# locuslab/lcp-physics

Measured on NVIDIA H100. Metric: LCP solves/sec (LCPFunction fwd+bwd, batch=4096 x 64 contacts, fp32), higher is better.
Workload: dtype f32 I/O and iterates; the condensed n x n KKT matrix is formed, factored and solved in f64

## Files before the change

lcp_physics_b200/csrc/lcp_condensed.cuh:

```cuda
#pragma once
#include "lcp_device.cuh"

namespace lcpb200 {
namespace cnd {

constexpr int NT = 256;
constexpr int UC = 8;
constexpr int CSMAX = 6;
constexpr int KS = 8;
constexpr int LMAX = 16;
constexpr int LU_BW = 2;
constexpr int MISC_BAND_LU = 4;
constexpr int CFLAG_DENSE_LU = 4;
constexpr int STATUS_UNSUPPORTED = -100;

struct CPlan {
  int ok;
  int n, m, e, N, NP, NS;
  int pcap;
  int wcap;
  int smem_bytes;
  int ctas_per_sm;
  int flags;
  int sbytes;
// ... 307 lines not shown
      S.clist()[rank * n + a] = (unsigned short)v;
    }
    if (l == 0) S.clcnt()[a] = (unsigned char)cnt;
  }
  __syncthreads();
  return true;
}

template <typename T>
struct EngineSoA {
  const T *mass, *inertia, *v, *fext;
  const T *normal, *p1, *p2;
  const T *mu, *rest;
  const int32_t *b1, *b2;
  const int32_t* nc_s;
  int nb, nc;
  int mode;
  T dt;
  T *p_s, *h_s;
};

template <typename T>
__device__ __forceinline__ void contact_row(T p1x, T p1y, T p2x, T p2y, T dx, T dy, T (&r1)[3], T (&r2)[3]) {
  r1[0] = p1x * dy - p1y * dx; r1[1] = dx; r1[2] = dy;
  r2[0] = -(p2x * dy - p2y * dx); r2[1] = -dx; r2[2] = -dy;
}

template <typename T>
__device__ __noinline__ bool build_structure_soa(const CPlan& P, CSmem<T>& S, Struct& st, const EngineSoA<T>& e_,
                                                 int sc, const T* __restrict__ A, int* singular) {
  const int n = P.n, e = P.e, tid = threadIdx.x, pcap = P.pcap;
  const int nb = e_.nb, ncs = e_.nc, cs = e_.mode == 0 ? 4 : 1;
  const int nc = e_.nc_s ? e_.nc_s[sc] : e_.nc;
  const int m = cs * nc;
  const int32_t* tb1 = e_.b1 + (e_.nc_s ? (size_t)sc * ncs : 0);
  const int32_t* tb2 = e_.b2 + (e_.nc_s ? (size_t)sc * ncs : 0);
  char* sb = reinterpret_cast<char*>(S.K());
  unsigned short* cl_tmp = reinterpret_cast<unsigned short*>(sb);
  int* cl_cnt = reinterpret_cast<int*>(sb + al16((size_t)LMAX * n * 2));
  if (n != 3 * nb || nc < 0 || nc > ncs || m > P.m || nc * cs > pcap || nc * cs * cs > P.wcap) return false;
  const T* mass = e_.mass + (size_t)sc * nb;
  const T* inertia = e_.inertia + (size_t)sc * nb;
  const T* v = e_.v + (size_t)sc * n;
  const T* normal = e_.normal + (size_t)sc * ncs * 2;
  const T* p1 = e_.p1 + (size_t)sc * ncs * 2;
  const T* p2 = e_.p2 + (size_t)sc * ncs * 2;
  T* ps = e_.p_s + (size_t)sc * n;
  T* hs = e_.h_s + (size_t)sc * P.m;
  int bad = 0;
  for (int j = tid; j < n; j += NT) {
    const int body = j / 3;
    const T q = (j - 3 * body == 0) ? inertia[body] : mass[body];
    S.qd()[j] = q;
    if (!(q != T(0) && isfinite((double)q))) bad |= 2;
    ps[j] = e_.mode == 0 ? q * v[j] + e_.dt * e_.fext[(size_t)sc * n + j] : T(0);
    cl_cnt[j] = 0;
  }
  for (int t = tid; t < e * n; t += NT) S.As()[t] = A[t];
  st.ncomp = nc; st.cs = cs; st.m = m;
  st.sh = 0;
  while ((1 << st.sh) < nc) ++st.sh;
  for (int t = tid; t < UC * pcap; t += NT) { S.Gd()[t] = T(0); S.ccols()[t] = 0; }
  for (int t = tid; t < nc * cs * cs; t += NT) S.Fd()[t] = T(0);
  __syncthreads();
  for (int c = tid; c < nc; c += NT) {
    const int b1 = tb1[c], b2 = tb2[c];
    if (b1 == b2 || b1 < 0 || b2 < 0 || b1 >= nb) { bad |= 1; continue; }
    const bool two = b2 < nb;
    const int lo = two ? min(b1, b2) : b1, hi = max(b1, b2);
    const int o1 = b1 < b2 ? 0 : 3, o2 = 3 - o1;
#pragma unroll
    for (int q = 0; q < 3; ++q) {
      S.ccols()[q * pcap + c] = (unsigned char)(3 * lo + q);
      if (two) S.ccols()[(3 + q) * pcap + c] = (unsigned char)(3 * hi + q);
    }
    S.ncols()[c] = two ? 6 : 3;
    const T nx = normal[2 * c], ny = normal[2 * c + 1];
    const T p1x = p1[2 * c], p1y = p1[2 * c + 1], p2x = p2[2 * c], p2y = p2[2 * c + 1];
    T r1[3], r2[3];
    contact_row<T>(p1x, p1y, p2x, p2y, nx, ny, r1, r2);
    const T v20 = two ? v[3 * b2] : T(0), v21 = two ? v[3 * b2 + 1] : T(0), v22 = two ? v[3 * b2 + 2] : T(0);
    const T jv = r1[0] * v[3 * b1] + r1[1] * v[3 * b1 + 1] + r1[2] * v[3 * b1 + 2] +
                 r2[0] * v20 + r2[1] * v21 + r2[2] * v22;
    const T rc = e_.rest[(size_t)sc * ncs + c];
#pragma unroll
    for (int q = 0; q < 3; ++q) { S.Gd()[(size_t)(o1 + q) * pcap + c] = r1[q]; if (two) S.Gd()[(size_t)(o2 + q) * pcap + c] = r2[q]; }
    S.rows()[c] = (unsigned short)c;
    S.posof()[c] = (unsigned short)c;
    if (e_.mode == 0) {
      hs[c] = jv * rc;
      contact_row<T>(p1x, p1y, p2x, p2y, ny, -nx, r1, r2);
#pragma unroll
      for (int q = 0; q < 3; ++q) {
        S.Gd()[(size_t)(o1 + q) * pcap + nc + c] = r1[q];
        S.Gd()[(size_t)(o1 + q) * pcap + 2 * nc + c] = -r1[q];
        if (two) { S.Gd()[(size_t)(o2 + q) * pcap + nc + c] = r2[q]; S.Gd()[(size_t)(o2 + q) * pcap + 2 * nc + c] = -r2[q]; }
      }
      const int rw[4] = {c, nc + 2 * c, nc + 2 * c + 1, 3 * nc + c};
#pragma unroll
      for (int r = 0; r < 4; ++r) { S.rows()[r * nc + c] = (unsigned short)rw[r]; S.posof()[rw[r]] = (unsigned short)(r * nc + c); }
      hs[nc + 2 * c] = T(0); hs[nc + 2 * c + 1] = T(0); hs[3 * nc + c] = T(0);
      S.Fd()[(size_t)(1 * 4 + 3) * nc + c] = T(1);
      S.Fd()[(size_t)(2 * 4 + 3) * nc + c] = T(1);
      S.Fd()[(size_t)(3 * 4 + 0) * nc + c] = e_.mu[(size_t)sc * ncs + c];
      S.Fd()[(size_t)(3 * 4 + 1) * nc + c] = T(-1);
      S.Fd()[(size_t)(3 * 4 + 2) * nc + c] = T(-1);
    } else {
      hs[c] = jv + jv * -rc;
    }
    for (int q = 0; q < (two ? 6 : 3); ++q) {
      const int a = q < 3 ? 3 * lo + q : 3 * hi + q - 3;
      const int slot = atomicAdd(&cl_cnt[a], 1);
      if (slot < LMAX) cl_tmp[slot * n + a] = (unsigned short)(c * 8 + q); else bad |= 1;
    }
  }
  const int anybad = __syncthreads_or(bad);
  if (anybad & 2) { *singular = 1; return false; }
  if (anybad & 1) return false;
  for (int t = tid; t < n * LMAX; t += NT) {
    const int a = t % n, l = t / n, cnt = cl_cnt[a];
    if (l < cnt) {
      const int val = cl_tmp[l * n + a];
      int rank = 0;
      for (int u = 0; u < cnt; ++u) rank += (cl_tmp[u * n + a] < val);
      S.clist()[rank * n + a] = (unsigned short)val;
    }
    if (l == 0) S.clcnt()[a] = (unsigned char)cnt;
  }
  __syncthreads();
  return true;
}

template <typename T>
__device__ __noinline__ void mark_band_lu(const CPlan& P, CSmem<T> S, Struct st) {
  int wide = P.e > 0 || (P.flags & CFLAG_DENSE_LU);
  for (int c = threadIdx.x; c < st.ncomp; c += NT) {
    const int nc = S.ncols()[c];
    if (nc > 0 && (S.ccols()[(nc - 1) * P.pcap + c] >> 4) - (S.ccols()[c] >> 4) > LU_BW) wide = 1;
  }
  wide = __syncthreads_or(wide);
  if (threadIdx.x == 0) S.misc()[MISC_BAND_LU] = !wide;
}

__device__ __forceinline__ double rcp64_fast(double x) {
  double r;
  asm("rcp.approx.ftz.f64 %0, %1;" : "=d"(r) : "d"(x));
  const double ax = fabs(x);
  if (!(ax > 1e-290 && ax < 1e290)) return 1.0 / x;
  r = fma(r, fma(-x, r, 1.0), r);
  r = fma(r, fma(-x, r, 1.0), r);
  return r;
}

template <typename T, int CS>
__device__ __forceinline__ void comp_inverse(const CPlan& P, CSmem<T>& S, const Struct& st) {
  const int nc_ = st.ncomp;
  for (int c = threadIdx.x; c < nc_; c += NT) {
    double M[CS][CS];
#pragma unroll
    for (int r = 0; r < CS; ++r) {
      const int i = S.rows()[r * nc_ + c];
#pragma unroll
      for (int q = 0; q < CS; ++q) M[r][q] = (double)S.Fd()[(size_t)(r * CS + q) * nc_ + c];
      M[r][r] += (i == 0xFFFF) ? 1.0 : ((P.flags & 1) ? 1.0 / (double)S.d()[i] : (double)(T(1) / S.d()[i]));
    }
    unsigned swaps = 0;
    int bit = 0;
#pragma unroll
    for (int k = 0; k < CS; ++k) {
#pragma unroll
      for (int i = k + 1; i < CS; ++i) {
        const bool sw = fabs(M[i][k]) > fabs(M[k][k]);
        swaps |= (sw ? 1u : 0u) << bit;
        ++bit;
#pragma unroll
        for (int q = 0; q < CS; ++q) { const double u = M[k][q], w = M[i][q]; M[k][q] = sw ? w : u; M[i][q] = sw ? u : w; }
      }
      const double r = rcp64_fast(M[k][k]);
      M[k][k] = 1.0;
#pragma unroll
      for (int q = 0; q < CS; ++q) M[k][q] *= r;
#pragma unroll
      for (int i = 0; i < CS; ++i) {
        if (i == k) continue;
        const double f = M[i][k];
        M[i][k] = 0.0;
#pragma unroll
        for (int q = 0; q < CS; ++q) M[i][q] = fma(-f, M[k][q], M[i][q]);
      }
    }
#pragma unroll
    for (int k = CS - 1; k >= 0; --k) {
#pragma unroll
      for (int i = CS - 1; i > k; --i) {
        --bit;
        const bool sw = (swaps >> bit) & 1u;
#pragma unroll
        for (int q = 0; q < CS; ++q) { const double u = M[q][k], w = M[q][i]; M[q][k] = sw ? w : u; M[q][i] = sw ? u : w; }
      }
    }
#pragma unroll
    for (int r = 0; r < CS; ++r)
#pragma unroll
      for (int q = 0; q < CS; ++q) S.W()[(size_t)(r * CS + q) * nc_ + c] = M[r][q];
  }
}

template <int CS>
struct ApplySpan {
  static constexpr int ceil_log2(int x) { return x <= 1 ? 0 : 1 + ceil_log2((x + 1) / 2); }
  static constexpr int U = ((CS << ceil_log2(4 * NT / CS)) + NT - 1) / NT;
};

template <typename T, int CS>
__device__ __forceinline__ void comp_apply(CSmem<T>& S, const Struct& st, bool trans = false) {
  constexpr int U = ApplySpan<CS>::U;
  const int nc_ = st.ncomp;
  const int npos = nc_ * CS;
  const int sh = st.sh, cmask = (1 << sh) - 1, tot = CS << sh;
  double val[U];
#pragma unroll
  for (int u = 0; u < U; ++u) {
    const int t = threadIdx.x + u * NT, r = t >> sh, c = t & cmask;
    val[u] = 0.0;
    if (t < tot && c < nc_) {
      double a = 0.0;
#pragma unroll
      for (int q = 0; q < CS; ++q) a = fma(S.W()[(size_t)(trans ? (q * CS + r) : (r * CS + q)) * nc_ + c], S.scr()[q * nc_ + c], a);
      val[u] = a;
    }
  }
  __syncthreads();
#pragma unroll
  for (int u = 0; u < U; ++u) {
    const int t = threadIdx.x + u * NT, r = t >> sh, c = t & cmask;
    if (t < tot && c < nc_) S.scr()[r * nc_ + c] = val[u];
  }
  (void)npos;
}

template <typename T, int NS, int CS>
__device__ __forceinline__ void assemble_K(const CPlan& P, CSmem<T>& S, const Struct& st) {
  const int nc_ = st.ncomp;
  constexpr int NP = 16 * NS;
  const int n = P.n, N = P.N, e = P.e, tid = threadIdx.x, pcap = P.pcap;
  double* K = S.K();
  {
    double2* K2 = reinterpret_cast<double2*>(K);
    for (int t = tid; t < NP * NP / 2; t += NT) K2[t] = make_double2(0.0, 0.0);
  }
  __syncthreads();
  for (int i = tid; i < NP; i += NT) K[(size_t)i * NP + i] = i < n ? (double)S.qd()[i] : (i < N ? 0.0 : 1.0);
  for (int t = tid; t < e * n; t += NT) {
    const int k = t / n, i = t - k * n;
    const double v = (double)S.As()[t];
    K[(size_t)(n + k) * NP + i] = v;
    K[(size_t)i * NP + n + k] = v;
  }
  __syncthreads();
  const int grp = tid >> 3, q2 = tid & 7;
  for (int a0 = 0; a0 < n; a0 += NT / 8) {
    const int a = a0 + grp;
    const int cnt = a < n ? (int)S.clcnt()[a] : 0;
    int mx = cnt;
    mx = max(mx, __shfl_xor_sync(FULL, mx, 8));
    mx = max(mx, __shfl_xor_sync(FULL, mx, 16));
    for (int l = 0; l < mx; ++l) {
      if (l < cnt) {
        const int cp = S.clist()[l * n + a], c = cp >> 3, p = cp & 7;
        if (q2 < (int)S.ncols()[c]) {
          double acc = 0.0;
#pragma unroll
          for (int q = 0; q < CS; ++q) {
            double u = 0.0;
#pragma unroll
            for (int r = 0; r < CS; ++r)
              u = fma((double)S.Gd()[(size_t)p * pcap + r * nc_ + c], S.W()[(size_t)(r * CS + q) * nc_ + c], u);
            acc = fma(u, (double)S.Gd()[(size_t)q2 * pcap + q * nc_ + c], acc);
          }
          K[(size_t)S.ccols()[q2 * pcap + c] * NP + a] += acc;
        }
      }
      __syncwarp();
    }
  }
  __syncthreads();
}

template <int NS, int BW>
struct LuBand {
  static constexpr bool DENSE = BW >= NS - 1;
  static constexpr int W = DENSE ? NS : 2 * BW + 1;
  static __device__ __forceinline__ constexpr bool in(int r, int c) { return DENSE || (r - c <= BW && c - r <= BW); }
  static __device__ __forceinline__ constexpr int col(int r, int c) { return DENSE ? c : c - r + BW; }
  static __host__ __device__ constexpr int end(int b0) { return DENSE || b0 + BW + 1 > NS ? NS : b0 + BW + 1; }
};

template <int NS, int BW, int B0>
__device__ __forceinline__ void lu_phase(double (&a)[NS][LuBand<NS, BW>::W], int o_buf, int o_rdiag, int& step, int ti,
                                         int tj) {
  using Bd = LuBand<NS, BW>;
  constexpr int NP = 16 * NS;
  constexpr int E = Bd::end(B0);
  constexpr int L = E - B0;
  constexpr int CW = (L <= 4) ? L : 3;
  double* const rdiag = reinterpret_cast<double*>(cnd_smem + o_rdiag);
#pragma unroll 1
  for (int kk = 0; kk < 16; kk += 2) {
    const int k = 16 * B0 + kk;
    double2* const U2 = reinterpret_cast<double2*>(cnd_smem + o_buf) + (size_t)(step & 1) * 2 * NP;
    double2* const C2 = U2 + NP;
    ++step;
    {
      const int sr = ti - kk, sc = tj - kk;
      if ((unsigned)sr < 2u) {
        double* dst = reinterpret_cast<double*>(U2) + sr;
#pragma unroll
        for (int c = B0; c < E; ++c) dst[2 * (16 * c + tj)] = a[B0][Bd::col(B0, c)];
      }
      if ((unsigned)sc < 2u) {
        double* dst = reinterpret_cast<double*>(C2) + sc;
#pragma unroll
        for (int r = B0; r < E; ++r) dst[2 * (16 * r + ti)] = a[r][Bd::col(r, B0)];
      }
    }
    __syncthreads();
    const double2 pk = U2[k], pk1 = U2[k + 1];
    const double p01 = pk1.x;
    const double r0 = rcp64_fast(pk.x);
    const double r1 = pk.x * rcp64_fast(fma(pk.x, pk1.y, -(pk.y * p01)));
    const double l10 = pk.y * r0;
    if ((ti | tj) == 0) { rdiag[k] = r0; rdiag[k + 1] = r1; }
#pragma unroll
    for (int cg = B0; cg < E; cg += CW) {
      double w0[CW], w1[CW];
#pragma unroll
      for (int q = 0; q < CW; ++q) {
        const int c = cg + q;
        if (c < E) {
          const double2 u = U2[16 * c + tj];
          const double x1 = fma(-l10, u.x, u.y);
          w0[q] = (c == B0 && !(tj > kk)) ? 0.0 : u.x;
          w1[q] = (c == B0 && !(tj > kk + 1)) ? 0.0 : x1;
        }
      }
#pragma unroll
      for (int r = B0; r < E; ++r) {
        const double2 cc = C2[16 * r + ti];
        double m0 = cc.x * r0;
        double m1 = fma(-m0, p01, cc.y) * r1;
        if (r == B0) {
          m0 = (ti > kk) ? m0 : 0.0;
          m1 = (ti > kk + 1) ? m1 : 0.0;
        }
#pragma unroll
        for (int q = 0; q < CW; ++q) {
          const int c = cg + q;
          if (c < E) a[r][Bd::col(r, c)] = fma(-m1, w1[q], fma(-m0, w0[q], a[r][Bd::col(r, c)]));
        }
      }
    }
  }
}

template <int NS, int BW, int B0>
struct LuPhases {
  static __device__ __forceinline__ void run(double (&a)[NS][LuBand<NS, BW>::W], int o_buf, int o_rdiag, int& step, int ti,
                                             int tj) {
    lu_phase<NS, BW, B0>(a, o_buf, o_rdiag, step, ti, tj);
    LuPhases<NS, BW, B0 + 1>::run(a, o_buf, o_rdiag, step, ti, tj);
  }
};
template <int NS, int BW>
struct LuPhases<NS, BW, NS> {
  static __device__ __forceinline__ void run(double (&)[NS][LuBand<NS, BW>::W], int, int, int&, int, int) {}
};

template <int NS> struct SolveLayout {
  static constexpr int NP = 16 * NS;
  static constexpr int QN = (NP + 31) / 32;
  static constexpr int ROUNDS = NP / QN;
  static constexpr size_t BYTES = (size_t)ROUNDS * QN * QN * 32 * 8;
};

template <int NS, int BW>
__device__ __forceinline__ void factor_K_body(int o_K, int o_rdiag, bool trans) {
  using Bd = LuBand<NS, BW>;
  constexpr int NP = 16 * NS, QN = SolveLayout<NS>::QN;
  int tid_;
  asm volatile("mov.u32 %0, %%tid.x;" : "=r"(tid_));
  const int ti = tid_ & 15, tj = tid_ >> 4;
  double* const K = reinterpret_cast<double*>(cnd_smem + o_K);
  double* const rdiag = reinterpret_cast<double*>(cnd_smem + o_rdiag);
  double a[NS][Bd::W];
#pragma unroll
  for (int c = 0; c < NS; ++c)
#pragma unroll
    for (int r = 0; r < NS; ++r)
      if (Bd::in(r, c)) a[r][Bd::col(r, c)] = K[(size_t)(16 * c + tj) * NP + 16 * r + ti];
  __syncthreads();
  int step = 0;
  LuPhases<NS, BW, 0>::run(a, o_K, o_rdiag, step, ti, tj);
  __syncthreads();
  int rowpart[NS];
  double rrow[NS];
#pragma unroll
  for (int r = 0; r < NS; ++r) {
    const int i = 16 * r + ti;
    rowpart[r] = trans ? (i / QN) * QN * QN * 32 + (i % QN) * 32 : (i % QN) * QN * 32 + i / QN;
    rrow[r] = rdiag[i];
  }
#pragma unroll
  for (int c = 0; c < NS; ++c) {
    const int j = 16 * c + tj;
    const double rj = rdiag[j];
    const int colpart = trans ? (j % QN) * QN * 32 + j / QN : (j / QN) * QN * QN * 32 + (j % QN) * 32;
#pragma unroll
    for (int r = 0; r < NS; ++r) {
      const int i = 16 * r + ti;
      const double v = Bd::in(r, c) ? a[r][Bd::col(r, c)] : 0.0;
      K[colpart + rowpart[r]] = (i != j) ? v * (trans ? rrow[r] : rj) : v;
    }
  }
  __syncthreads();
}

template <int NS>
__device__ __noinline__ void factor_K(int o_K, int o_rdiag, bool trans, bool band) {
  if constexpr (LU_BW < NS - 1) {
    if (band) {
      factor_K_body<NS, LU_BW>(o_K, o_rdiag, trans);
      return;
    }
  }
  factor_K_body<NS, NS - 1>(o_K, o_rdiag, trans);
}

template <int QN>
struct SolveCoef {
  double dg[QN * QN];
  double rw[QN * QN];
};

template <int QN>
__device__ __forceinline__ void solve_load(SolveCoef<QN>& c, const double* blk, int r, int lane) {
#pragma unroll
  for (int t = 0; t < QN * QN; ++t) { c.dg[t] = blk[t * 32 + r]; c.rw[t] = blk[t * 32 + lane]; }
}

template <int QN>
__device__ __forceinline__ void solve_round_fwd(double (&y)[QN], const SolveCoef<QN>& c, int r, int lane) {
  double v[QN];
#pragma unroll
  for (int q = 0; q < QN; ++q) v[q] = __shfl_sync(FULL, y[q], r);
#pragma unroll
  for (int q = 0; q < QN; ++q)
#pragma unroll
    for (int qp = q + 1; qp < QN; ++qp) v[qp] = fma(-c.dg[qp * QN + q], v[q], v[qp]);
  const bool below = lane > r, own = lane == r;
#pragma unroll
  for (int qp = 0; qp < QN; ++qp) {
    double t = y[qp];
#pragma unroll
    for (int q = 0; q < QN; ++q) t = fma(-c.rw[qp * QN + q], v[q], t);
    y[qp] = below ? t : (own ? v[qp] : y[qp]);
  }
}

template <int QN>
__device__ __forceinline__ void solve_round_bwd(double (&y)[QN], const SolveCoef<QN>& c, int r, int lane) {
  double v[QN];
#pragma unroll
  for (int q = 0; q < QN; ++q) v[q] = __shfl_sync(FULL, y[q], r);
#pragma unroll
  for (int q = QN - 1; q >= 0; --q)
#pragma unroll
    for (int qp = q - 1; qp >= 0; --qp) v[qp] = fma(-c.dg[qp * QN + q], v[q], v[qp]);
  const bool above = lane < r, own = lane == r;
#pragma unroll
  for (int qp = 0; qp < QN; ++qp) {
    double t = y[qp];
#pragma unroll
    for (int q = QN - 1; q >= 0; --q) t = fma(-c.rw[qp * QN + q], v[q], t);
    y[qp] = above ? t : (own ? v[qp] : y[qp]);
  }
}

template <int NS>
__device__ __noinline__ void solve_warp(int o_K, int o_rdiag, int o_bx) {
  constexpr int NP = 16 * NS, QN = SolveLayout<NS>::QN, ROUNDS = SolveLayout<NS>::ROUNDS;
  constexpr int STRIDE = QN * QN * 32;
  static_assert(ROUNDS % 2 == 0, "the software pipeline handles two rounds per trip");
  const int lane = threadIdx.x & 31;
  const double* const S = reinterpret_cast<const double*>(cnd_smem + o_K);
  const double* const rdiag = reinterpret_cast<const double*>(cnd_smem + o_rdiag);
  double* const bx = reinterpret_cast<double*>(cnd_smem + o_bx);
  double y[QN];
#pragma unroll
  for (int q = 0; q < QN; ++q) y[q] = (QN * lane + q < NP) ? bx[QN * lane + q] : 0.0;
  SolveCoef<QN> c0, c1;
  solve_load<QN>(c0, S, 0, lane);
#pragma unroll 1
  for (int r = 0; r < ROUNDS; r += 2) {
    solve_load<QN>(c1, S + (size_t)(r + 1) * STRIDE, r + 1, lane);
    solve_round_fwd<QN>(y, c0, r, lane);
    const int rn = (r + 2 < ROUNDS) ? r + 2 : ROUNDS - 1;
    solve_load<QN>(c0, S + (size_t)rn * STRIDE, rn, lane);
    solve_round_fwd<QN>(y, c1, r + 1, lane);
  }
#pragma unroll 1
  for (int r = ROUNDS - 1; r > 0; r -= 2) {
    solve_load<QN>(c1, S + (size_t)(r - 1) * STRIDE, r - 1, lane);
    solve_round_bwd<QN>(y, c0, r, lane);
    const int rn = (r - 2 >= 0) ? r - 2 : 0;
    solve_load<QN>(c0, S + (size_t)rn * STRIDE, rn, lane);
    solve_round_bwd<QN>(y, c1, r - 1, lane);
  }
#pragma unroll
  for (int q = 0; q < QN; ++q) {
    const int i = QN * lane + q;
    if (i < NP) bx[i] = y[q] * rdiag[i];
  }
}

template <typename T, int CS, int NS, typename PF>
__device__ __noinline__ void solve_kkt(const CPlan& P, CSmem<T> S, Struct st, PF& pf, const T* rx,
                                       const T* rs, const T* rz, const T* ry, T* dx, T* ds, T* dz, T* dy,
                                       bool trans = false) {
  const int nc_ = st.ncomp;
  const int n = P.n, e = P.e, N = P.N, NP = P.NP, tid = threadIdx.x, pcap = P.pcap;
  const int npos = st.ncomp * CS;
  for (int p = tid; p < npos; p += NT) {
    const int i = S.rows()[p];
    double t = 0.0;
    if (i != 0xFFFF) t = (P.flags & 2) ? ((double)(rz ? rz[i] : T(0)) - (double)rs[i] / (double)S.d()[i]) : (double)((rz ? rz[i] : T(0)) - rs[i] / S.d()[i]);
    S.scr()[p] = t;
  }
  __syncthreads();
  comp_apply<T, CS>(S, st, trans);
  __syncthreads();
  for (int a = tid; a < NP; a += NT) {
    double acc = 0.0;
    if (a < n) {
      const int cnt = S.clcnt()[a];
      for (int l = 0; l < cnt; ++l) {
        const int cp = S.clist()[l * n + a], c = cp >> 3, p = cp & 7;
#pragma unroll
        for (int r = 0; r < CS; ++r) acc = fma((double)S.Gd()[(size_t)p * pcap + r * nc_ + c], S.scr()[r * nc_ + c], acc);
      }
      acc = -(double)(rx ? rx[a] : T(0)) - acc;
    } else if (a < N) {
      acc = -(double)(ry ? ry[a - n] : T(0));
    }
    S.bx()[a] = acc;
  }
  __syncthreads();
  pf.lap(CPH_SOLVE_RHS);
  if (tid < 32) solve_warp<NS>(P.o_K, P.o_rdiag, P.o_bx);
  __syncthreads();
  pf.lap(CPH_SOLVE_TRI);
  for (int tt = tid; tt < (CS << st.sh); tt += NT) {
    const int c = tt & ((1 << st.sh) - 1);
    if (c >= nc_) continue;
    const int p = (tt >> st.sh) * nc_ + c;
    const int i = S.rows()[p];
    double t = 0.0;
    if (i != 0xFFFF) {
      const int nc = S.ncols()[c];
      t = (P.flags & 2) ? ((double)(rz ? rz[i] : T(0)) - (double)rs[i] / (double)S.d()[i]) : (double)((rz ? rz[i] : T(0)) - rs[i] / S.d()[i]);
      for (int q = 0; q < nc; ++q) t = fma((double)S.Gd()[(size_t)q * pcap + p], S.bx()[S.ccols()[q * pcap + c]], t);
    }
    S.scr()[p] = t;
  }
  __syncthreads();
  comp_apply<T, CS>(S, st, trans);
  __syncthreads();
  for (int p = tid; p < npos; p += NT) {
    const int i = S.rows()[p];
    if (i == 0xFFFF) continue;
    const T wz = (T)S.scr()[p];
    const T rsi = rs[i];
    dz[i] = wz;
    ds[i] = (-rsi - wz) / S.d()[i];
  }
  for (int a = tid; a < n; a += NT) dx[a] = (T)S.bx()[a];
  for (int k = tid; k < e; k += NT) dy[k] = (T)S.bx()[n + k];
  __syncthreads();
  pf.lap(CPH_SOLVE_POST);
}

template <typename T, int NS, int CS, typename PF>
__device__ __noinline__ void factor_kkt(const CPlan& P, CSmem<T> S, Struct st, PF& pf, bool trans = false) {
  comp_inverse<T, CS>(P, S, st);
  __syncthreads();
  pf.lap(CPH_WINV);
  assemble_K<T, NS, CS>(P, S, st);
  pf.lap(CPH_ASSEMBLE);
  if constexpr (LU_BW < NS - 1) factor_K<NS>(P.o_K, P.o_rdiag, trans, S.misc()[MISC_BAND_LU] != 0);
  else factor_K<NS>(P.o_K, P.o_rdiag, trans, false);
  pf.lap(CPH_LU);
}

template <typename T>
__device__ __forceinline__ void get_steps(const T* z, const T* dz, const T* s, const T* ds, int m, T* red, T& step_z,
                                          T& step_s) {
  const T NEG_INF = -INFINITY, POS_INF = INFINITY;
  T mx[2] = {NEG_INF, NEG_INF};
  T mn[2] = {POS_INF, POS_INF};
  T any[2] = {T(0), T(0)};
  for (int i = threadIdx.x; i < m; i += NT) {
    const T az = -z[i] / dz[i], as = -s[i] / ds[i];
    mx[0] = nan_max(mx[0], az);
    mx[1] = nan_max(mx[1], as);
    if (dz[i] > T(0)) any[0] = T(1); else mn[0] = nan_min(mn[0], az);
    if (ds[i] > T(0)) any[1] = T(1); else mn[1] = nan_min(mn[1], as);
  }
  T v[6] = {mx[0], mx[1], -mn[0], -mn[1], any[0], any[1]};
  block_reduce<T, 6>(v, OpMax(), NEG_INF, red);
  const T fz = (v[0] > T(1)) ? v[0] : T(1);
  const T fs = (v[1] > T(1)) ? v[1] : T(1);
  step_z = (v[4] > T(0)) ? nan_min(-v[2], fz) : -v[2];
  step_s = (v[5] > T(0)) ? nan_min(-v[3], fs) : -v[3];
}

template <typename T>
struct CFwdArgs {
  CPlan P;
  int B;
  const T *Q, *p, *G, *h, *A, *b, *F;
  T *zhat, *nu, *lam, *slack, *resid;
  int *status, *iters;
  T eps;
  int not_improved_lim, max_iter;
  long long* prof;
  EngineSoA<T> soa;
  unsigned char* ssave;
};

template <typename T>
struct CBwdArgs {
  CPlan P;
  int B;
  int R, chunks;
  const T *Q, *G, *A, *F;
  const T *zhat, *nu, *lam, *slack, *g;
  T *dQ, *dp, *dG, *dh, *dA, *db, *dF;
  int* done;
  const int* only;
  unsigned flags;
  const unsigned char* sload;
  EngineSoA<T> soa;
  T *dmass, *dinertia, *dv, *dfext, *dnormal, *dp1, *dp2, *dmu, *drest;
  long long* prof;
};

__device__ __forceinline__ void copy16(unsigned char* dst, const unsigned char* src, int bytes) {
  const uint4* s4 = reinterpret_cast<const uint4*>(src);
  uint4* d4 = reinterpret_cast<uint4*>(dst);
  for (int i = threadIdx.x; i < (bytes >> 4); i += NT) d4[i] = s4[i];
}

__device__ __forceinline__ void save_structure(const CPlan& P, const Struct& st, bool ok, unsigned char* dst) {
  if (threadIdx.x == 0) *reinterpret_cast<int4*>(dst) = make_int4(ok ? st.ncomp : -1, st.cs, st.sh, st.m);
  if (!ok) return;
  const int c1 = P.o_x - P.o_Fd, c2 = P.o_y - P.o_qd, c3 = P.o_misc - P.o_rows;
  copy16(dst + 16, cnd_smem + P.o_Fd, c1);
  copy16(dst + 16 + c1, cnd_smem + P.o_qd, c2);
  copy16(dst + 16 + c1 + c2, cnd_smem + P.o_rows, c3);
}

__device__ __forceinline__ bool load_structure(const CPlan& P, Struct& st, const unsigned char* src) {
  const int4 hd = *reinterpret_cast<const int4*>(src);
  st.ncomp = hd.x; st.cs = hd.y; st.sh = hd.z; st.m = hd.w;
  if (hd.x < 0) return false;
  const int c1 = P.o_x - P.o_Fd, c2 = P.o_y - P.o_qd, c3 = P.o_misc - P.o_rows;
  copy16(cnd_smem + P.o_Fd, src + 16, c1);
  copy16(cnd_smem + P.o_qd, src + 16 + c1, c2);
  copy16(cnd_smem + P.o_rows, src + 16 + c1 + c2, c3);
  return true;
}

template <typename T>
struct SzResid { T sz, resid; };

template <typename T, int CS>
__device__ __noinline__ SzResid<T> fwd_residuals(const CFwdArgs<T>& a, CSmem<T> S, Struct st, int sc) {
  const int nc_ = st.ncomp;
  const CPlan& P = a.P;
  const int n = P.n, m = st.m, e = P.e, tid = threadIdx.x, pcap = P.pcap;
  const T* p = a.p + (size_t)sc * n;
  const T* h = a.h + (size_t)sc * P.m;
  const T* b = e > 0 ? a.b + (size_t)sc * e : nullptr;
  for (int c = tid; c < n; c += NT) {
    T acc = 0;
    const int cnt = S.clcnt()[c];
    for (int l = 0; l < cnt; ++l) {
      const int cp = S.clist()[l * n + c], cc = cp >> 3, pp = cp & 7;
#pragma unroll
      for (int r = 0; r < CS; ++r) {
        const int i = S.rows()[r * nc_ + cc];
        if (i != 0xFFFF) acc = fma(S.Gd()[(size_t)pp * pcap + r * nc_ + cc], S.z()[i], acc);
      }
    }
    for (int k = 0; k < e; ++k) acc = fma(S.As()[k * n + c], S.y()[k], acc);
    S.rx()[c] = acc + S.qd()[c] * S.x()[c] + p[c];
  }
  for (int tt = tid; tt < (CS << st.sh); tt += NT) {
    const int r = tt >> st.sh, c = tt & ((1 << st.sh) - 1);
    if (c >= nc_) continue;
    const int pz = r * nc_ + c;
    const int i = S.rows()[pz];
    if (i == 0xFFFF) continue;
    const int nc = S.ncols()[c];
    T acc = 0;
    for (int q = 0; q < nc; ++q) acc = fma(S.Gd()[(size_t)q * pcap + pz], S.x()[S.ccols()[q * pcap + c]], acc);
    T fz = 0;
#pragma unroll
    for (int q = 0; q < CS; ++q) {
      const int j = S.rows()[q * nc_ + c];
      if (j != 0xFFFF) fz = fma(S.Fd()[(size_t)(r * CS + q) * nc_ + c], S.z()[j], fz);
    }
    S.rz()[i] = acc + S.s()[i] - h[i] - fz;
  }
  for (int k = tid; k < e; k += NT) {
    T acc = 0;
    for (int j = 0; j < n; ++j) acc = fma(S.As()[k * n + j], S.x()[j], acc);
    S.ry()[k] = acc - b[k];
  }
  __syncthreads();
  T q4[4] = {0, 0, 0, 0};
  for (int i = tid; i < m; i += NT) { q4[0] += S.s()[i] * S.z()[i]; q4[1] += S.rz()[i] * S.rz()[i]; }
  for (int i = tid; i < e; i += NT) q4[2] += S.ry()[i] * S.ry()[i];
  for (int i = tid; i < n; i += NT) q4[3] += S.rx()[i] * S.rx()[i];
  block_reduce<T, 4>(q4, OpSum(), T(0), S.red());
  const T sz = q4[0];
  const T mu = fabs(sz / T(m));
  return {sz, (e > 0 ? sqrt(q4[2]) : T(0)) + sqrt(q4[1]) + sqrt(q4[3]) + T(m) * mu};
}

template <typename T>
__device__ __noinline__ void fwd_store_best(const CFwdArgs<T>& a, CSmem<T> S, int m, int sc) {
  const CPlan& P = a.P;
  const int n = P.n, e = P.e, tid = threadIdx.x;
  for (int i = tid; i < n; i += NT) a.zhat[(size_t)sc * n + i] = S.x()[i];
  for (int i = tid; i < m; i += NT) { a.lam[(size_t)sc * P.m + i] = S.z()[i]; a.slack[(size_t)sc * P.m + i] = S.s()[i]; }
  for (int i = tid; i < e; i += NT) a.nu[(size_t)sc * e + i] = S.y()[i];
}

template <typename T>
__device__ __noinline__ void fwd_centering(CSmem<T> S, int m, T mu, T sz) {
  const int tid = threadIdx.x;
  T stz, sts;
  get_steps(S.z(), S.dz(), S.s(), S.ds(), m, S.red(), stz, sts);
  const T alpha_aff = nan_min(nan_min(stz, sts), T(1));
  T t3[1] = {0};
  for (int i = tid; i < m; i += NT) t3[0] += (S.s()[i] + alpha_aff * S.ds()[i]) * (S.z()[i] + alpha_aff * S.dz()[i]);
  block_reduce<T, 1>(t3, OpSum(), T(0), S.red());
  const T ratio = t3[0] / sz;
  const T sig = ratio * ratio * ratio;
  const T musig = -mu * sig;
  for (int i = tid; i < m; i += NT) S.rs2()[i] = (musig + S.ds()[i] * S.dz()[i]) / S.s()[i];
  __syncthreads();
}

template <typename T>
__device__ __noinline__ void fwd_step(const CPlan& P, CSmem<T> S, int m) {
  const int n = P.n, e = P.e, tid = threadIdx.x;
  for (int i = tid; i < n; i += NT) S.dx()[i] += S.rx()[i];
  for (int i = tid; i < m; i += NT) { S.ds()[i] += S.rz()[i]; S.dz()[i] += S.rs2()[i]; }
  for (int i = tid; i < e; i += NT) S.dy()[i] += S.ry()[i];
  __syncthreads();
  T stz, sts;
  get_steps(S.z(), S.dz(), S.s(), S.ds(), m, S.red(), stz, sts);
  const T alpha = nan_min(T(0.999) * nan_min(stz, sts), T(1));
  for (int i = tid; i < n; i += NT) S.x()[i] += alpha * S.dx()[i];
  for (int i = tid; i < m; i += NT) { S.s()[i] += alpha * S.ds()[i]; S.z()[i] += alpha * S.dz()[i]; }
  for (int i = tid; i < e; i += NT) S.y()[i] += alpha * S.dy()[i];
  __syncthreads();
}

template <typename T, int NS, int CS, typename PF>
__device__ __forceinline__ void forward_scene(const CFwdArgs<T>& a, CSmem<T>& S, const Struct& st, PF& pf, int sc) {
  const CPlan& P = a.P;
  const int m = st.m;
  {
    const int n = P.n, e = P.e, tid = threadIdx.x;
    const T* h = a.h + (size_t)sc * P.m;
    const T* b = e > 0 ? a.b + (size_t)sc * e : nullptr;
    for (int i = tid; i < m; i += NT) { S.d()[i] = T(1); S.rs2()[i] = T(0); S.rz()[i] = -h[i]; }
    for (int i = tid; i < n; i += NT) S.rx()[i] = a.p[(size_t)sc * n + i];
    for (int i = tid; i < e; i += NT) S.ry()[i] = -b[i];
    __syncthreads();
  }
  factor_kkt<T, NS, CS>(P, S, st, pf);
  solve_kkt<T, CS, NS>(P, S, st, pf, S.rx(), S.rs2(), S.rz(), P.e > 0 ? S.ry() : nullptr, S.x(), S.s(), S.z(), S.y());
  if (m == 0) {
    fwd_store_best<T>(a, S, 0, sc);
    if (threadIdx.x == 0) { a.status[sc] = 2; a.iters[sc] = 0; if (a.resid) a.resid[sc] = T(0); }
    return;
  }
  {
    const int tid = threadIdx.x;
    T mn[2] = {INFINITY, INFINITY};
    for (int i = tid; i < m; i += NT) { mn[0] = nan_min(mn[0], S.s()[i]); mn[1] = nan_min(mn[1], S.z()[i]); }
    block_reduce<T, 2>(mn, OpMin(), (T)INFINITY, S.red());
    for (int i = tid; i < m; i += NT) {
      if (mn[0] <= T(0)) S.s()[i] -= mn[0] - T(1);
      if (mn[1] <= T(0)) S.z()[i] -= mn[1] - T(1);
    }
    __syncthreads();
  }

  T best = nan("");
  bool have_best = false;
  int not_improved = 0, status = 0, it = 0;
  for (it = 0; it < a.max_iter; ++it) {
    const SzResid<T> r = fwd_residuals<T, CS>(a, S, st, sc);
    pf.lap(CPH_RESID);
    const T mu = fabs(r.sz / T(m));

    bool improved;
    if (!have_best) { improved = true; have_best = true; not_improved = 0; }
    else { improved = r.resid < best; not_improved = improved ? 0 : not_improved + 1; }
    if (improved) {
      best = r.resid;
      fwd_store_best<T>(a, S, m, sc);
    }
    if (not_improved == a.not_improved_lim) { status = 1; ++it; break; }
    if (best < a.eps) { status = 2; ++it; break; }
    if (mu > T(1e100)) { status = 3; ++it; break; }

    for (int i = threadIdx.x; i < m; i += NT) S.d()[i] = S.z()[i] / S.s()[i];
    __syncthreads();
    factor_kkt<T, NS, CS>(P, S, st, pf);

    solve_kkt<T, CS, NS>(P, S, st, pf, S.rx(), S.z(), S.rz(), P.e > 0 ? S.ry() : nullptr, S.dx(), S.ds(), S.dz(), S.dy());
    fwd_centering<T>(S, m, mu, r.sz);
    pf.lap(CPH_STEP);
    solve_kkt<T, CS, NS>(P, S, st, pf, nullptr, S.rs2(), nullptr, nullptr, S.rx(), S.rz(), S.rs2(), S.ry());
    fwd_step<T>(P, S, m);
    pf.lap(CPH_STEP);
  }
  if (threadIdx.x == 0) { a.status[sc] = status; a.iters[sc] = it; if (a.resid) a.resid[sc] = best; }
}

template <typename T, int NS, bool PROF>
__global__ void __launch_bounds__(NT, (NS <= 6) ? 2 : 1) cond_forward_kernel(const __grid_constant__ CFwdArgs<T> a) {
  const CPlan& P = a.P;
  CSmem<T> S(P);
  const int n = P.n, m = P.m, e = P.e, tid = threadIdx.x;
  __shared__ int singular_s;
  const T NANV = nan("");
  Prof<PROF> pf(PROF ? a.prof + (size_t)blockIdx.x * CPH_COUNT : nullptr);
  for (int sc = blockIdx.x; sc < a.B; sc += gridDim.x) {
    if (tid == 0) singular_s = 0;
    __syncthreads();
    pf.start();
    Struct st;
    const bool ok = a.soa.mass
        ? build_structure_soa<T>(P, S, st, a.soa, sc, e > 0 ? a.A + (size_t)sc * e * n : nullptr, &singular_s)
        : build_structure<T>(P, S, st, a.Q + (size_t)sc * n * n, a.G + (size_t)sc * m * n,
                             e > 0 ? a.A + (size_t)sc * e * n : nullptr, a.F + (size_t)sc * m * m, &singular_s);
    __syncthreads();
    if (a.ssave) save_structure(P, st, ok, a.ssave + (size_t)sc * P.sbytes);
    pf.lap(CPH_STRUCT);
    if (!ok) {
      if (singular_s) {
        for (int i = tid; i < n; i += NT) a.zhat[(size_t)sc * n + i] = NANV;
        for (int i = tid; i < m; i += NT) { a.lam[(size_t)sc * m + i] = NANV; a.slack[(size_t)sc * m + i] = NANV; }
        for (int i = tid; i < e; i += NT) a.nu[(size_t)sc * e + i] = NANV;
        if (tid == 0) { a.status[sc] = -1; a.iters[sc] = 0; if (a.resid) a.resid[sc] = NANV; }
      } else if (tid == 0) {
        a.status[sc] = STATUS_UNSUPPORTED;
        a.iters[sc] = 0;
      }
      __syncthreads();
      continue;
    }
    if constexpr (LU_BW < NS - 1) mark_band_lu<T>(P, S, st);
    switch (st.cs) {
      case 1: forward_scene<T, NS, 1>(a, S, st, pf, sc); break;
      case 2: forward_scene<T, NS, 2>(a, S, st, pf, sc); break;
      case 3: forward_scene<T, NS, 3>(a, S, st, pf, sc); break;
      case 4: forward_scene<T, NS, 4>(a, S, st, pf, sc); break;
      case 5: forward_scene<T, NS, 5>(a, S, st, pf, sc); break;
      default: forward_scene<T, NS, 6>(a, S, st, pf, sc); break;
    }
    __syncthreads();
  }
}

template <typename T, typename F>
__device__ __forceinline__ void write_outer(T* __restrict__ o, int rows, int cols, F f) {
  constexpr int V = 16 / (int)sizeof(T);
  const int tid = threadIdx.x;
  if (cols % V == 0 && (reinterpret_cast<size_t>(o) & 15) == 0) {
    const int cv = cols / V, total = rows * cv;
    const int di = NT / cv, dj = NT - di * cv;
    int i = tid / cv, jv = tid - i * cv;
    for (int t = tid; t < total; t += NT) {
      const int j = jv * V;
      if (V == 4) {
        float4 w;
        w.x = (float)f(i, j); w.y = (float)f(i, j + 1); w.z = (float)f(i, j + 2); w.w = (float)f(i, j + 3);
        reinterpret_cast<float4*>(o)[t] = w;
      } else {
        double2 w;
        w.x = (double)f(i, j); w.y = (double)f(i, j + 1);
        reinterpret_cast<double2*>(o)[t] = w;
      }
      i += di; jv += dj;
      if (jv >= cv) { jv -= cv; ++i; }
    }
  } else {
    int i = tid / cols, j = tid - i * cols;
    const int di = NT / cols, dj = NT - di * cols;
    for (size_t t = tid; t < (size_t)rows * cols; t += NT) {
      o[t] = f(i, j);
      i += di; j += dj;
      if (j >= cols) { j -= cols; ++i; }
    }
  }
}

template <typename T, int CS, typename PF>
__device__ __forceinline__ void backward_grads(const CBwdArgs<T>& a, CSmem<T>& S, const Struct& st, PF& pf, int sc, int so) {
  const CPlan& P = a.P;
  const int n = P.n, m = st.m, e = P.e, tid = threadIdx.x;
  const T* dx = S.dx(); const T* dlam = S.dz(); const T* dnu = S.dy();
  if (a.soa.mass) {
    const EngineSoA<T>& E = a.soa;
    const int nc = st.ncomp, nb = E.nb, ncs = E.nc;
    const int32_t* tb1 = E.b1 + (E.nc_s ? (size_t)sc * ncs : 0);
    const int32_t* tb2 = E.b2 + (E.nc_s ? (size_t)sc * ncs : 0);
    const T* v = E.v + (size_t)sc * n;
    const T* zh_ = S.x(); const T* lm = S.z();
    for (int c = tid; c < ncs; c += NT) {
      const size_t ic = (size_t)sc * ncs + c, oc = (size_t)so * ncs + c;
      if (c >= nc) {
        if (a.dnormal) { a.dnormal[oc * 2] = 0; a.dnormal[oc * 2 + 1] = 0; }
        if (a.dp1) { a.dp1[oc * 2] = 0; a.dp1[oc * 2 + 1] = 0; }
        if (a.dp2) { a.dp2[oc * 2] = 0; a.dp2[oc * 2 + 1] = 0; }
        if (a.drest) a.drest[oc] = 0;
        if (a.dmu) a.dmu[oc] = 0;
        continue;
      }
      const T nx = E.normal[ic * 2], ny = E.normal[ic * 2 + 1];
      const T p1x = E.p1[ic * 2], p1y = E.p1[ic * 2 + 1], p2x = E.p2[ic * 2], p2y = E.p2[ic * 2 + 1];
      const bool two = tb2[c] < nb;
      const int j1 = 3 * tb1[c], j2 = two ? 3 * tb2[c] : j1;
      const T rc = E.rest[ic];
      const T dhc = -dlam[c] * (E.mode == 0 ? T(1) : T(1));
      T gnx = 0, gny = 0, g1x = 0, g1y = 0, g2x = 0, g2y = 0, jcv = 0;
      const int nrows = E.mode == 0 ? 3 : 1;
      const int rows_[3] = {c, nc + 2 * c, nc + 2 * c + 1};
      const T dxs[3] = {nx, ny, -ny}, dys[3] = {ny, -nx, nx};
      for (int q = 0; q < nrows; ++q) {
        const T ddx_ = dxs[q], ddy_ = dys[q];
        const int i = rows_[q];
        T g[6];
        for (int t = 0; t < 3; ++t) {
          g[t] = dlam[i] * zh_[j1 + t] + lm[i] * dx[j1 + t];
          g[3 + t] = two ? dlam[i] * zh_[j2 + t] + lm[i] * dx[j2 + t] : T(0);
        }
        if (q == 0) {
          const T row[6] = {p1x * ddy_ - p1y * ddx_, ddx_, ddy_, -(p2x * ddy_ - p2y * ddx_), -ddx_, -ddy_};
          for (int t = 0; t < 3; ++t) jcv += row[t] * v[j1 + t] + row[3 + t] * (two ? v[j2 + t] : T(0));
          const T hs_ = E.mode == 0 ? rc : (T(1) - rc);
          for (int t = 0; t < 3; ++t) { g[t] += dhc * hs_ * v[j1 + t]; g[3 + t] += dhc * hs_ * (two ? v[j2 + t] : T(0)); }
        }
        const T gdx = -p1y * g[0] + g[1] + p2y * g[3] - g[4];
        const T gdy = p1x * g[0] + g[2] - p2x * g[3] - g[5];
        g1x += ddy_ * g[0]; g1y += -ddx_ * g[0];
        g2x += -ddy_ * g[3]; g2y += ddx_ * g[3];
        if (q == 0) { gnx += gdx; gny += gdy; }
        else if (q == 1) { gny += gdx; gnx += -gdy; }
        else { gny += -gdx; gnx += gdy; }
      }
      if (a.dnormal) { a.dnormal[oc * 2] = gnx; a.dnormal[oc * 2 + 1] = gny; }
      if (a.dp1) { a.dp1[oc * 2] = g1x; a.dp1[oc * 2 + 1] = g1y; }
      if (a.dp2) { a.dp2[oc * 2] = g2x; a.dp2[oc * 2 + 1] = g2y; }
      if (a.drest) a.drest[oc] = E.mode == 0 ? dhc * jcv : -dhc * jcv;
      if (a.dmu) a.dmu[oc] = E.mode == 0 ? -(dlam[3 * nc + c] * lm[c]) : T(0);
    }
    for (int j = tid; j < n; j += NT) {
      const int body = j / 3, comp = j - 3 * body;
      const T md = comp == 0 ? E.inertia[(size_t)sc * nb + body] : E.mass[(size_t)sc * nb + body];
// ... 125 lines not shown
```

Baseline: 303,800.

## Parallelize per-component inverse and apply across warp lanes with shuffles

Changes the per-component small dense inverse from one thread per component to one lane per row, with a group of CS lanes per component. Pivot rows are exchanged with warp shuffles. The block-diagonal apply is fused into the RHS and back-substitution loops through shuffles, which removes the shared-memory scratch round trip and several block barriers. The d=z/s update is folded into the inverse, and a barrier in fwd_step is dropped. This raises parallelism in the small-matrix phases at the cost of shuffle traffic and some idle lanes when 32 is not a multiple of CS. Removing the fwd_step barrier risks a race if get_steps reads values written by other threads before it synchronizes internally.

New measurement: 310,000 (median of 6 runs). 2.0% higher.

```diff
diff --git a/lcp_physics_b200/csrc/lcp_condensed.cuh b/lcp_physics_b200/csrc/lcp_condensed.cuh
--- a/lcp_physics_b200/csrc/lcp_condensed.cuh
+++ b/lcp_physics_b200/csrc/lcp_condensed.cuh
@@ -483,41 +483,83 @@
   return r;
 }
 
+template <int CS>
+struct CompLanes {
+  static constexpr int GPW = 32 / CS;
+  static constexpr int STEP = GPW * (NT / 32);
+  int r;
+  int lead;
+  int c0;
+  __device__ __forceinline__ CompLanes() {
+    const int lane = threadIdx.x & 31, g = lane / CS;
+    r = lane - g * CS;
+    lead = g * CS;
+    c0 = g < GPW ? (int)(threadIdx.x >> 5) * GPW + g : 1 << 30;
+  }
+  __device__ __forceinline__ double row(double v, int q) const { return __shfl_sync(FULL, v, lead + q); }
+};
+
 template <typename T, int CS>
-__device__ __forceinline__ void comp_inverse(const CPlan& P, CSmem<T>& S, const Struct& st) {
+__device__ __forceinline__ void comp_inverse(const CPlan& P, CSmem<T>& S, const Struct& st, bool d_zs) {
   const int nc_ = st.ncomp;
-  for (int c = threadIdx.x; c < nc_; c += NT) {
-    double M[CS][CS];
-#pragma unroll
-    for (int r = 0; r < CS; ++r) {
-      const int i = S.rows()[r * nc_ + c];
-#pragma unroll
-      for (int q = 0; q < CS; ++q) M[r][q] = (double)S.Fd()[(size_t)(r * CS + q) * nc_ + c];
-      M[r][r] += (i == 0xFFFF) ? 1.0 : ((P.flags & 1) ? 1.0 / (double)S.d()[i] : (double)(T(1) / S.d()[i]));
+  const CompLanes<CS> L;
+  for (int cb = 0; cb < nc_; cb += CompLanes<CS>::STEP) {
+    const int c = cb + L.c0;
+    const bool own = c < nc_;
+    double M[CS];
+#pragma unroll
+    for (int q = 0; q < CS; ++q) M[q] = own ? (double)S.Fd()[(size_t)(L.r * CS + q) * nc_ + c] : 0.0;
+    if (own) {
+      const int i = S.rows()[L.r * nc_ + c];
+      double dg = 1.0;
+      if (i != 0xFFFF) {
+        T d;
+        if (d_zs) {
+          d = S.z()[i] / S.s()[i];
+          S.d()[i] = d;
+        } else {
+          d = S.d()[i];
+        }
+        dg = (P.flags & 1) ? 1.0 / (double)d : (double)(T(1) / d);
+      }
+#pragma unroll
+      for (int q = 0; q < CS; ++q)
+        if (q == L.r) M[q] += dg;
     }
     unsigned swaps = 0;
     int bit = 0;
 #pragma unroll
     for (int k = 0; k < CS; ++k) {
+      double col[CS];
+#pragma unroll
+      for (int i = k; i < CS; ++i) col[i] = L.row(M[k], i);
+      double piv = col[k];
+      int src_k = k, src = L.r;
 #pragma unroll
       for (int i = k + 1; i < CS; ++i) {
-        const bool sw = fabs(M[i][k]) > fabs(M[k][k]);
+        const bool sw = fabs(col[i]) > fabs(piv);
         swaps |= (sw ? 1u : 0u) << bit;
         ++bit;
-#pragma unroll
-        for (int q = 0; q < CS; ++q) { const double u = M[k][q], w = M[i][q]; M[k][q] = sw ? w : u; M[i][q] = sw ? u : w; }
-      }
-      const double r = rcp64_fast(M[k][k]);
-      M[k][k] = 1.0;
-#pragma unroll
-      for (int q = 0; q < CS; ++q) M[k][q] *= r;
-#pragma unroll
-      for (int i = 0; i < CS; ++i) {
-        if (i == k) continue;
-        const double f = M[i][k];
-        M[i][k] = 0.0;
-#pragma unroll
-        for (int q = 0; q < CS; ++q) M[i][q] = fma(-f, M[k][q], M[i][q]);
+        if (sw && L.r == i) src = src_k;
+        if (sw) { src_k = i; piv = col[i]; }
+      }
+      if (L.r == k) src = src_k;
+      const double rk = rcp64_fast(piv);
+      double pr[CS];
+#pragma unroll
+      for (int q = 0; q < CS; ++q) {
+        const double mine = L.row(M[q], src), pv = L.row(M[q], src_k);
+        M[q] = mine;
+        pr[q] = (q == k ? 1.0 : pv) * rk;
+      }
+      if (L.r == k) {
+#pragma unroll
+        for (int q = 0; q < CS; ++q) M[q] = pr[q];
+      } else {
+        const double f = M[k];
+        M[k] = 0.0;
+#pragma unroll
+        for (int q = 0; q < CS; ++q) M[q] = fma(-f, pr[q], M[q]);
       }
     }
 #pragma unroll
@@ -526,48 +568,28 @@
       for (int i = CS - 1; i > k; --i) {
         --bit;
         const bool sw = (swaps >> bit) & 1u;
-#pragma unroll
-        for (int q = 0; q < CS; ++q) { const double u = M[q][k], w = M[q][i]; M[q][k] = sw ? w : u; M[q][i] = sw ? u : w; }
-      }
-    }
-#pragma unroll
-    for (int r = 0; r < CS; ++r)
-#pragma unroll
-      for (int q = 0; q < CS; ++q) S.W()[(size_t)(r * CS + q) * nc_ + c] = M[r][q];
-  }
-}
-
-template <int CS>
-struct ApplySpan {
-  static constexpr int ceil_log2(int x) { return x <= 1 ? 0 : 1 + ceil_log2((x + 1) / 2); }
-  static constexpr int U = ((CS << ceil_log2(4 * NT / CS)) + NT - 1) / NT;
-};
+        const double u = M[k], w = M[i];
+        M[k] = sw ? w : u;
+        M[i] = sw ? u : w;
+      }
+    }
+    if (own) {
+#pragma unroll
+      for (int q = 0; q < CS; ++q) S.W()[(size_t)(L.r * CS + q) * nc_ + c] = M[q];
+    }
+  }
+}
 
 template <typename T, int CS>
-__device__ __forceinline__ void comp_apply(CSmem<T>& S, const Struct& st, bool trans = false) {
-  constexpr int U = ApplySpan<CS>::U;
-  const int nc_ = st.ncomp;
-  const int npos = nc_ * CS;
-  const int sh = st.sh, cmask = (1 << sh) - 1, tot = CS << sh;
-  double val[U];
-#pragma unroll
-  for (int u = 0; u < U; ++u) {
-    const int t = threadIdx.x + u * NT, r = t >> sh, c = t & cmask;
-    val[u] = 0.0;
-    if (t < tot && c < nc_) {
-      double a = 0.0;
-#pragma unroll
-      for (int q = 0; q < CS; ++q) a = fma(S.W()[(size_t)(trans ? (q * CS + r) : (r * CS + q)) * nc_ + c], S.scr()[q * nc_ + c], a);
-      val[u] = a;
-    }
-  }
-  __syncthreads();
-#pragma unroll
-  for (int u = 0; u < U; ++u) {
-    const int t = threadIdx.x + u * NT, r = t >> sh, c = t & cmask;
-    if (t < tot && c < nc_) S.scr()[r * nc_ + c] = val[u];
-  }
-  (void)npos;
+__device__ __forceinline__ double comp_apply(const CSmem<T>& S, const CompLanes<CS>& L, int nc_, int c, bool own, double v,
+                                             bool trans) {
+  double a = 0.0;
+#pragma unroll
+  for (int q = 0; q < CS; ++q) {
+    const double w = own ? S.W()[(size_t)(trans ? (q * CS + L.r) : (L.r * CS + q)) * nc_ + c] : 0.0;
+    a = fma(w, L.row(v, q), a);
+  }
+  return a;
 }
 
 template <typename T, int NS, int CS>
@@ -860,15 +882,23 @@
                                        bool trans = false) {
   const int nc_ = st.ncomp;
   const int n = P.n, e = P.e, N = P.N, NP = P.NP, tid = threadIdx.x, pcap = P.pcap;
-  const int npos = st.ncomp * CS;
-  for (int p = tid; p < npos; p += NT) {
-    const int i = S.rows()[p];
+  const CompLanes<CS> L;
+  auto rhs_t = [&](int i) -> double {
+    return (P.flags & 2) ? ((double)(rz ? rz[i] : T(0)) - (double)rs[i] / (double)S.d()[i])
+                         : (double)((rz ? rz[i] : T(0)) - rs[i] / S.d()[i]);
+  };
+  for (int cb = 0; cb < nc_; cb += CompLanes<CS>::STEP) {
+    const int c = cb + L.c0;
+    const bool own = c < nc_;
+    const int p = L.r * nc_ + c;
     double t = 0.0;
-    if (i != 0xFFFF) t = (P.flags & 2) ? ((double)(rz ? rz[i] : T(0)) - (double)rs[i] / (double)S.d()[i]) : (double)((rz ? rz[i] : T(0)) - rs[i] / S.d()[i]);
-    S.scr()[p] = t;
-  }
-  __syncthreads();
-  comp_apply<T, CS>(S, st, trans);
+    if (own) {
+      const int i = S.rows()[p];
+      if (i != 0xFFFF) t = rhs_t(i);
+    }
+    const double wt = comp_apply<T, CS>(S, L, nc_, c, own, t, trans);
+    if (own) S.scr()[p] = wt;
+  }
   __syncthreads();
   for (int a = tid; a < NP; a += NT) {
     double acc = 0.0;
@@ -890,29 +920,24 @@
   if (tid < 32) solve_warp<NS>(P.o_K, P.o_rdiag, P.o_bx);
   __syncthreads();
   pf.lap(CPH_SOLVE_TRI);
-  for (int tt = tid; tt < (CS << st.sh); tt += NT) {
-    const int c = tt & ((1 << st.sh) - 1);
-    if (c >= nc_) continue;
-    const int p = (tt >> st.sh) * nc_ + c;
-    const int i = S.rows()[p];
+  for (int cb = 0; cb < nc_; cb += CompLanes<CS>::STEP) {
+    const int c = cb + L.c0;
+    const bool own = c < nc_;
+    const int p = L.r * nc_ + c;
+    const int i = own ? S.rows()[p] : 0xFFFF;
     double t = 0.0;
     if (i != 0xFFFF) {
       const int nc = S.ncols()[c];
-      t = (P.flags & 2) ? ((double)(rz ? rz[i] : T(0)) - (double)rs[i] / (double)S.d()[i]) : (double)((rz ? rz[i] : T(0)) - rs[i] / S.d()[i]);
+      t = rhs_t(i);
       for (int q = 0; q < nc; ++q) t = fma((double)S.Gd()[(size_t)q * pcap + p], S.bx()[S.ccols()[q * pcap + c]], t);
     }
-    S.scr()[p] = t;
-  }
-  __syncthreads();
-  comp_apply<T, CS>(S, st, trans);
-  __syncthreads();
-  for (int p = tid; p < npos; p += NT) {
-    const int i = S.rows()[p];
-    if (i == 0xFFFF) continue;
-    const T wz = (T)S.scr()[p];
-    const T rsi = rs[i];
-    dz[i] = wz;
-    ds[i] = (-rsi - wz) / S.d()[i];
+    const double w = comp_apply<T, CS>(S, L, nc_, c, own, t, trans);
+    if (i != 0xFFFF) {
+      const T wz = (T)w;
+      const T rsi = rs[i];
+      dz[i] = wz;
+      ds[i] = (-rsi - wz) / S.d()[i];
+    }
   }
   for (int a = tid; a < n; a += NT) dx[a] = (T)S.bx()[a];
   for (int k = tid; k < e; k += NT) dy[k] = (T)S.bx()[n + k];
@@ -921,8 +946,8 @@
 }
 
 template <typename T, int NS, int CS, typename PF>
-__device__ __noinline__ void factor_kkt(const CPlan& P, CSmem<T> S, Struct st, PF& pf, bool trans = false) {
-  comp_inverse<T, CS>(P, S, st);
+__device__ __noinline__ void factor_kkt(const CPlan& P, CSmem<T> S, Struct st, PF& pf, bool trans = false, bool d_zs = false) {
+  comp_inverse<T, CS>(P, S, st, d_zs);
   __syncthreads();
   pf.lap(CPH_WINV);
   assemble_K<T, NS, CS>(P, S, st);
@@ -1100,7 +1125,6 @@
   for (int i = tid; i < n; i += NT) S.dx()[i] += S.rx()[i];
   for (int i = tid; i < m; i += NT) { S.ds()[i] += S.rz()[i]; S.dz()[i] += S.rs2()[i]; }
   for (int i = tid; i < e; i += NT) S.dy()[i] += S.ry()[i];
-  __syncthreads();
   T stz, sts;
   get_steps(S.z(), S.dz(), S.s(), S.ds(), m, S.red(), stz, sts);
   const T alpha = nan_min(T(0.999) * nan_min(stz, sts), T(1));
@@ -1161,9 +1185,7 @@
     if (best < a.eps) { status = 2; ++it; break; }
     if (mu > T(1e100)) { status = 3; ++it; break; }
 
-    for (int i = threadIdx.x; i < m; i += NT) S.d()[i] = S.z()[i] / S.s()[i];
-    __syncthreads();
-    factor_kkt<T, NS, CS>(P, S, st, pf);
+    factor_kkt<T, NS, CS>(P, S, st, pf, false, true);
 
     solve_kkt<T, CS, NS>(P, S, st, pf, S.rx(), S.z(), S.rz(), P.e > 0 ? S.ry() : nullptr, S.dx(), S.ds(), S.dz(), S.dy());
     fwd_centering<T>(S, m, mu, r.sz);
```
